# skitzoid/Box2D-MT

Measured on AMD Instinct MI355X. Metric: world steps/sec at 99858 bodies per GPU (BASELINE config 3: Tumbler 100k, CCD off; Step = collide + island solve + broad-phase + state read-back); for N > 1: container-steps/s = world steps/s x N containers in the one sharded world, higher is better.
Workload: dtype f32

## Files before the change

box2d-mt_amd/csrc/b2d_kernels_broadphase.h:

```cpp
#ifndef B2D_KERNELS_BROADPHASE_H
#define B2D_KERNELS_BROADPHASE_H

#include "b2d_kernels_solve_large.h"

#define SYNC_TILE 1024
__global__ __launch_bounds__(256) void k_sync_fixtures(DW W)
{
	b2dPhaseStamp(W);
	DState* S = W.st;
	const int n = W.nProxies;
	const int tid = (int)threadIdx.x;
	__shared__ int s_list[SYNC_TILE];
	__shared__ int s_cnt, s_base;
	const int perLane = n >= 262144 ? SYNC_TILE / 256 : 1, tile = 256 * perLane;
	if (blockIdx.x == 0 && tid == 0) S->c.gridFresh = 0;
	for (int base = blockIdx.x * tile; base < n; base += gridDim.x * tile)
	{
		if (tid == 0) s_cnt = 0;
		__syncthreads();
		for (int j = 0; j < perLane; ++j)
		{
			const int p = base + j * 256 + tid;
			if (p >= n) break;
			const int body = W.p_body[p];
// ... 638 lines not shown
__device__ __forceinline__ bool createBlocked(const DW& W, const DState* S, int smallPath)
{
	if (smallPath && S->c.nPairs > COUNT_RANK_MAX) return true;
	if (!smallPath && (S->c.overflow & 2) != 0) return true;
	return S->c.nContacts + S->c.nNewContacts > W.capContacts;
}

__global__ __launch_bounds__(256) void k_create_contacts(DW W, const uint64_t* keys, const int2* proxies, int smallPath)
{
	b2dPhaseStamp(W);
	DState* S = W.st;
	const int n = S->c.nPairs < W.capPairs ? S->c.nPairs : W.capPairs;
	if (createBlocked(W, S, smallPath)) return;
	const int base = S->c.nContacts;
	const ContactArrays& C = W.ca[S->cur];
	for (int i = blockIdx.x * blockDim.x + threadIdx.x; i < n; i += gridDim.x * blockDim.x)
	{
		if (!W.pairFirst[i]) continue;
		const int dst = base + W.pairRank[i];
		if (dst >= W.capContacts)
		{
			atomicOr(&S->c.overflow, 1);
			continue;
		}
		int2 pr = proxies[i];
		int pA = pr.x, pB = pr.y;
		if (b2dContactSwap(W.shapes[W.p_shape[pA]].type, W.shapes[W.p_shape[pB]].type) == 1)
		{
			int t = pA;
			pA = pB;
// ... 1 lines not shown
		}
		const int bodyA = W.p_body[pA], bodyB = W.p_body[pB];
		const bool sensor = ((W.p_filter1[pA] | W.p_filter1[pB]) & PF_SENSOR) != 0;
		uint32_t flags = CF_ENABLED | (sensor ? CF_SENSOR : 0u);
		if (isToiCandidate(W, pA, pB, bodyA, bodyB))
		{
			flags |= CF_TOI_CANDIDATE;
			const int k = atomicAdd(&S->c.nNewToiCand, 1);
			if (k < TOI_NEW_LIST_MAX) W.toiNewList[k] = dst;
		}
		float2 mA = W.p_mat[pA], mB = W.p_mat[pB];
		float friction = b2dSqrt(mA.x * mB.x);
		float restitution = mA.y > mB.y ? mA.y : mB.y;
		C.ids[dst] = make_int4(pA, pB, bodyA, bodyB);
		C.key[dst] = keys[i];
		C.flags[dst] = flags;
		C.mat[dst] = make_float4(friction, restitution, 0.0f, 1.0f);
		C.man0[dst] = make_float4(0, 0, 0, 0);
		C.man1[dst] = make_float4(0, 0, 0, 0);
		C.imp[dst] = make_float4(0, 0, 0, 0);
		C.man3[dst] = make_int4(0, 0, 0, 0);
		C.color[dst] = -1;
		C.mgr[dst] = -1;
		if (!sensor)
		{
			W.b_wake[bodyA] = 1;
			W.b_wake[bodyB] = 1;
		}
	}
}

__global__ __launch_bounds__(256) void k_create_finish(DW W, int smallPath)
{
	b2dPhaseStamp(W);
	DState* S = W.st;
	if (createBlocked(W, S, smallPath)) return;
	for (int i = blockIdx.x * blockDim.x + threadIdx.x; i < W.nBodies; i += gridDim.x * blockDim.x)
	{
		if (W.b_wake[i])
		{
			W.b_wake[i] = 0;
			const uint32_t f = W.b_flags[i];
			if ((f & BF_AWAKE) != 0 && W.b_pos[i].w == 0.0f) continue;
			W.b_flags[i] = f | BF_AWAKE;
// ... 257 lines not shown
```

box2d-mt_amd/csrc/b2d_kernels_collide.h:

```cpp
#ifndef B2D_KERNELS_COLLIDE_H
#define B2D_KERNELS_COLLIDE_H

#include "b2d_world.h"
#include "b2d_toi.h"

__device__ __forceinline__ Xf loadXf(const float4* b_xf, int body)
{
	float4 t = b_xf[body];
	Xf xf;
	xf.p = v2(t.x, t.y);
	xf.q.s = t.z;
	xf.q.c = t.w;
	return xf;
}

__device__ __forceinline__ AABB loadAabb(const float4* p_fat, int proxy)
{
	float4 t = p_fat[proxy];
	AABB a;
	a.lo = v2(t.x, t.y);
	a.hi = v2(t.z, t.w);
	return a;
}

// ... 690 lines not shown
	for (int i = blockIdx.x * blockDim.x + threadIdx.x; i < n; i += gridDim.x * blockDim.x)
	{
		const int4 ids = C.ids[i];
		const unsigned lo = (unsigned)(ids.z < ids.w ? ids.z : ids.w), hi = (unsigned)(ids.z < ids.w ? ids.w : ids.z);
		const unsigned long long key = ((unsigned long long)lo << 32) | hi;
		int a = 0, b = nPairs;
		while (a < b)
		{
			const int m = (a + b) >> 1;
			if (pairs[m] < key) a = m + 1; else b = m;
		}
		if (a < nPairs && pairs[a] == key) C.flags[i] |= CF_FILTER;
	}
}

__global__ __launch_bounds__(256) void k_compact_contacts(DW W)
{
	b2dPhaseStamp(W);
	DState* S = W.st;
	if (S->c.nDestroy == 0) return;
	const int n = S->c.nContacts;
	const ContactArrays& A = W.ca[S->cur];
	const ContactArrays& B = W.ca[1 - S->cur];
	for (int i = blockIdx.x * blockDim.x + threadIdx.x; i < n; i += gridDim.x * blockDim.x)
	{
		if (W.keepFlag[i])
		{
			int j = W.keepScan[i];
			const uint32_t fl = A.flags[i];
			B.ids[j] = A.ids[i];
			B.key[j] = A.key[i];
			B.flags[j] = fl;
			if ((fl & CF_FOREIGN) == 0)
			{
				B.mat[j] = A.mat[i];
				B.man0[j] = A.man0[i];
				B.man1[j] = A.man1[i];
				B.imp[j] = A.imp[i];
				B.man3[j] = A.man3[i];
			}
			B.color[j] = A.color[i];
			const int m = A.mgr[i];
			B.mgr[j] = m;
			if (m >= 0) W.toiPos2c[m] = j;
		}
	}
	if (b2dLastBlockArrive(W, ARRIVE_COMPACT) && threadIdx.x == 0)
	{
		S->c.nContacts = W.keepScan[n];
		S->cur = 1 - S->cur;
	}
}

__device__ __forceinline__ uint32_t hashKey(uint64_t k)
{
	k ^= k >> 33;
	k *= 0xff51afd7ed558ccdULL;
	k ^= k >> 33;
	k *= 0xc4ceb9fe1a85ec53ULL;
	k ^= k >> 33;
	return (uint32_t)k;
}

__device__ __forceinline__ uint32_t htLiveMask(const DW& W)
{
	const uint32_t want = 4u * (uint32_t)W.st->c.nContacts + 1024u;
	uint32_t m = 0xffffffffu >> __clz((int)(want | 1u));
	return m < W.htMask ? m : W.htMask;
}

__device__ __forceinline__ void htInsert(const DW& W, uint64_t key)
{
	const uint32_t mask = htLiveMask(W);
	uint32_t h = hashKey(key) & mask;
	for (;;)
	{
		unsigned long long old = atomicCAS((unsigned long long*)&W.ht_keys[h], 0ull, (unsigned long long)key);
		if (old == 0ull || old == key) return;
		h = (h + 1) & mask;
	}
}

__device__ __forceinline__ bool htContains(const DW& W, uint64_t key)
{
	const uint32_t mask = htLiveMask(W);
	uint32_t h = hashKey(key) & mask;
	for (;;)
	{
		uint64_t v = W.ht_keys[h];
		if (v == key) return true;
		if (v == 0) return false;
		h = (h + 1) & mask;
	}
}

__global__ __launch_bounds__(256) void k_ht_clear(DW W)
{
	b2dPhaseStamp(W);
	if (W.st->c.nMoves == 0) return;
	for (uint32_t i = blockIdx.x * blockDim.x + threadIdx.x, live = htLiveMask(W); i <= live; i += gridDim.x * blockDim.x)
	{
		W.ht_keys[i] = 0;
	}
}

__global__ __launch_bounds__(256) void k_ht_build(DW W)
{
	b2dPhaseStamp(W);
	DState* S = W.st;
	if (S->c.nMoves == 0) return;
	const int n = S->c.nContacts;
	const ContactArrays& C = W.ca[S->cur];
	for (int i = blockIdx.x * blockDim.x + threadIdx.x; i < n; i += gridDim.x * blockDim.x)
	{
		htInsert(W, C.key[i] + 1ull);
	}
}

#endif
```

box2d-mt_amd/csrc/b2d_kernels_toi.h:

```cpp
#ifndef B2D_KERNELS_TOI_H
#define B2D_KERNELS_TOI_H

#include "b2d_kernels_broadphase.h"
#include "b2d_toi.h"

#define TOI_LANES 512
#define TOI_CAND_MAX 512
#define TOI_MOVES_MAX 128
#define TOI_PAIRS_MAX 512
#define TOI_RECOMP_MAX 512
#define TOI_WOKEN_MAX 256
#define TOI_EVENTS_MAX 100000
#define TOI_NEWPAIR_MAX 256
#define TOI_MOVED_ALL_MAX 32768

__device__ __forceinline__ uint32_t ldFlags(const uint32_t* p)
{
	return __hip_atomic_load(p, __ATOMIC_RELAXED, __HIP_MEMORY_SCOPE_AGENT);
}

__device__ __forceinline__ Sweep loadSweep(const DW& W, int body)
{
	const float4 p0 = W.b_pos0[body], p = W.b_pos[body], m = W.b_mass[body];
	Sweep s;
// ... 1133 lines not shown
		for (int i = tid; i < nPairs; i += LANES)
		{
			if (!s_pairFirst[i] || !s_pairCand[i] || base + s_pairRank[i] >= W.capContacts) continue;
			int before = 0;
			for (int j = 0; j < nPairs; ++j)
			{
				if (s_pairFirst[j] && s_pairCand[j] && s_pairRank[j] < s_pairRank[i]) ++before;
			}
			const int slot = s_toiOrder + before;
			C.mgr[base + s_pairRank[i]] = slot;
			W.toiPos2c[slot] = base + s_pairRank[i];
		}
		__syncthreads();
		if (tid == 0)
		{
			int total = s_nC + s_nNew;
			if (total > W.capContacts) total = W.capContacts;
			s_nC = total;
			s_events += 1;
			int cands = 0;
			for (int j = 0; j < nPairs; ++j) cands += (s_pairFirst[j] && s_pairCand[j] && base + s_pairRank[j] < W.capContacts) ? 1 : 0;
			s_toiOrder += cands;
		}
		__syncthreads();

		}
		const int nB = solid ? s_nBodies : 0;
		TOI_T(7);
		const int nTail = s_nC - nC0;
		for (int bi = 0; bi < nB; ++bi)
// ... 94 lines not shown
```

box2d-mt_amd/csrc/b2d_kernels_toi_chains.h:

```cpp
#ifndef B2D_KERNELS_TOI_CHAINS_H
#define B2D_KERNELS_TOI_CHAINS_H

#include "b2d_kernels_toi.h"

#define CHAIN_LANES 64
#define CHAIN_CAND_MAX 64
#define CHAIN_EVENTS_MAX 4096
#define CHAIN_ADJ_MAX 32
#define TOI_GROUPS_MAX 262144

#define TOI_UNSAFE_PARTNER 1
#define TOI_UNSAFE_WOKE 2
#define TOI_UNSAFE_PAIR 4
#define TOI_UNSAFE_CAPACITY 8
#define TOI_UNSAFE_MOVED 16

__global__ __launch_bounds__(256) void k_toi_groups_begin(DW W)
{
	b2dPhaseStamp(W);
	DState* S = W.st;
	const int n = S->c.nToiList < W.capContacts ? S->c.nToiList : W.capContacts;
	const ContactArrays& C = W.ca[S->cur];
	for (int k = blockIdx.x * blockDim.x + threadIdx.x; k < n; k += gridDim.x * blockDim.x)
	{
// ... 127 lines not shown
			A.mat[i] = B.mat[i];
			A.man0[i] = B.man0[i];
			A.man1[i] = B.man1[i];
			A.imp[i] = B.imp[i];
			A.man3[i] = B.man3[i];
		}
		if (t0 == 0)
		{
			S->c.nToiEvents = 0;
			S->c.nToiMoved = 0;
			S->c.nToiNewPairs = 0;
			S->c.nToiChainCreated = 0;
			S->c.nToiLog = 0;
			S->c.toiIncomplete = 0;
			S->c.spToiStraddle = 0;
			S->c.nContacts = S->c.nContactsSnap;
			S->c.nToiOrder = S->c.nToiOrderSnap;
		}
	}
}

__device__ __forceinline__ void toiChainRun(const DW& W, const StepParams& sp, int haveGrid, int group, int* census)
{
	DState* S = W.st;
	const ContactArrays& C = W.ca[S->cur];
	const int lane = threadIdx.x;
	const int D = W.toiGroups[group];
	const int* adjL = W.toiGroupList + (size_t)group * CHAIN_ADJ_MAX;
	const int nAdj = W.toiGroupCount[group] < CHAIN_ADJ_MAX ? W.toiGroupCount[group] : CHAIN_ADJ_MAX;
	const float4 massD = W.b_mass[D];
// ... 578 lines not shown
				C.color[dst] = -1;
				C.mgr[dst] = -1;
				if (!sensor)
				{
					W.b_pos[bodyA].w = 0.0f;
					W.b_pos[bodyB].w = 0.0f;
					W.b_rowDirty[bodyA] = 1;
					W.b_rowDirty[bodyB] = 1;
				}
			}
			__syncthreads();
			if (threadIdx.x == 0)
			{
				S->c.nContacts = base + s_created;
				S->c.nToiChainCreated = s_created;
			}
		}
	}
}

__global__ __launch_bounds__(CHAIN_LANES) void k_toi_chains(DW W, StepParams sp, int haveGrid)
{
	b2dPhaseStamp(W);
	DState* S = W.st;
	__shared__ int s_chainCensus[2];
	if (threadIdx.x == 0) { s_chainCensus[0] = 0; s_chainCensus[1] = 0; }
	__syncthreads();
	if ((S->c.toiUnsafe & (TOI_UNSAFE_PARTNER | TOI_UNSAFE_CAPACITY)) == 0)
	{
		const int nGroups = S->c.nToiGroups < TOI_GROUPS_MAX ? S->c.nToiGroups : TOI_GROUPS_MAX;
// ... 7 lines not shown
	if (b2dLastBlockArrive(W, ARRIVE_CHAINS, (unsigned)s_chainCensus[0], (unsigned)s_chainCensus[1], &events, &calls))
	{
		if (threadIdx.x == 0)
		{
			if (events) atomicAdd(&S->c.nToiEvents, (int)events);
			if (calls) atomicAdd(&S->c.nToiCalls, (int)calls);
		}
		toiChainsEnd(W);
	}
}

__global__ __launch_bounds__(256) void k_bp_clear(DW W)
{
	b2dPhaseStamp(W);
	DState* S = W.st;
	if (blockIdx.x == 0 && threadIdx.x == 0)
	{
		S->c.nLargeProxies = 0;
		S->c.nLargeMoves = 0;
		S->c.nPairs = 0;
		S->c.nNewContacts = 0;
		S->c.nMovesSeen = S->c.nMoves;
		S->c.gridFresh = S->c.nMoves != 0 ? 1 : 0;
	}
	if (blockIdx.x == 0 && threadIdx.x < 32) S->c.candRounds[threadIdx.x] = 0;
	if (S->c.nMoves == 0) return;
	const uint32_t stride = gridDim.x * blockDim.x, t0 = blockIdx.x * blockDim.x + threadIdx.x;
	{
		const float cap = 4.0f * W.cellSize;
		float ext = 0.0f;
		for (uint32_t p = t0; p < (uint32_t)W.nProxies; p += stride)
		{
// ... 1 lines not shown
			const float4 a = W.p_fat[p];
			const float e = fmaxf(a.z - a.x, a.w - a.y);
			if (e <= cap && e > ext) ext = e;
		}
		blockAtomicMaxIfAbove((int*)&S->c.cellExtBits, ext > 0.0f ? (int)__float_as_uint(ext) : 0);
	}
	{
		const int4 z = make_int4(0, 0, 0, 0);
		int4* gc = (int4*)W.gridCount;
		int4* gu = (int4*)W.gridCursor;
		for (uint32_t i = t0, n4 = (W.gridMask + 1u) >> 2; i < n4; i += stride)
		{
			gc[i] = z;
			gu[i] = z;
		}
		int4* hk = (int4*)W.ht_keys;
		for (uint32_t i = t0, n2 = (htLiveMask(W) + 1u) >> 1; i < n2; i += stride) hk[i] = z;
	}
}

__global__ __launch_bounds__(256) void k_bp_build(DW W)
{
	b2dPhaseStamp(W);
	DState* S = W.st;
	if (S->c.nMoves == 0) return;
	const int stride = gridDim.x * blockDim.x, t0 = blockIdx.x * blockDim.x + threadIdx.x;
	const int nC = S->c.nContacts;
	const ContactArrays& C = W.ca[S->cur];
	for (int i = t0; i < nC; i += stride) if ((C.flags[i] & CF_FOREIGN) == 0) htInsert(W, C.key[i] + 1ull);
	const int n = W.nProxies;
	for (int p = t0; p < n; p += stride)
	{
		if (W.p_body[p] < 0) continue;
		const float4 a = W.p_fat[p];
		if (proxyIsLarge(W, a))
		{
			const int k = atomicAdd(&S->c.nLargeProxies, 1);
			W.largeProxies[k] = p;
		}
		else
		{
			int ix, iy;
			proxyCell(W, a, &ix, &iy);
			atomicAdd(&W.gridCount[cellHash(ix, iy, W.gridMask)], 1);
// ... 6 lines not shown
```

box2d-mt_amd/csrc/b2d_world.h:

```cpp
#ifndef B2D_WORLD_H
#define B2D_WORLD_H

#include "b2d_solver.h"
#include "b2d_joint.h"
#include "b2d_wave.h"

#define BF_TYPE_MASK 0x3u
#define BF_AWAKE 0x4u
#define BF_AUTOSLEEP 0x8u
#define BF_BULLET 0x10u
#define BF_FIXEDROT 0x20u
#define BF_ACTIVE 0x40u
#define BF_ISLAND 0x80u
#define BF_LARGE 0x100u

#define BT_STATIC 0u
#define BT_KINEMATIC 1u
#define BT_DYNAMIC 2u

#define CF_TOUCHING 0x1u
#define CF_ENABLED 0x2u
#define CF_FILTER 0x4u
#define CF_TOI_CANDIDATE 0x8u
#define CF_SENSOR 0x10u
// ... 141 lines not shown
	int collideBlocksDone;
	int chainBlocksDone;
	int edgesBlocksDone;
	int nFreeIslands;
	int nSmallJointed;
	int nStraddle;
	int nStraddleJoints;
	int nResolve;
	int nMigrated;
	int spContacts[SHARD_MAX_RANKS], spJoints[SHARD_MAX_RANKS];
	int spMigBodies[SHARD_MAX_RANKS];
	int spBodies[SHARD_MAX_RANKS], spProxies[SHARD_MAX_RANKS];
	int spToiCreated;
	int spToiStraddle;
	int spOwnRows;
};

struct PreSolveRec
{
	int4 info;
	unsigned long long key;
	unsigned long long pad;
	float4 o0, o1, oimp;
	int4 o3;
	float4 n0, n1, nimp;
	int4 n3;
	float4 mat;
};
struct ToiLogRec
{
// ... 38 lines not shown
struct DW
{
	DState* st;
	uint32_t stampMask;
	int nBodies, nProxies, nJoints, nShapes;
	int capContacts, capPairs, capMoves;
	int serialOrphans;
	int noFreeBodies;
	int testMaxColors, testColorRounds;
	int testSpinMax;
	int restPoll;
	int hubSerial;
	int smallMaxW;
	int bigChunks;
	uint32_t htMask;
	uint32_t gridMask;
	float cellSize, invCellSize;

	float4* b_pos;
	float4* b_pos0;
	float4* b_vel;
	float4* b_xf;
	float4* b_mass;
	float4* b_damp;
	float4* b_force;
	uint32_t* b_flags;
	int* b_wake;
	int* b_order;
	int* orderBody;

// ... 320 lines not shown
```

box2d-mt_amd/csrc/b2hip_api_callbacks.h:

```cpp

int b2hip_set_contact_filter(b2hip_world* w, b2hip_should_collide_fn fn, void* user)
{
	if (int rcu = checkUsable(w, "b2hip_set_contact_filter", true)) return rcu;
	w->filterFn = fn;
	w->filterUser = user;
	w->dw.userFilter = hasFilter(w) ? 1 : 0;
	return B2HIP_OK;
}

int b2hip_set_contact_filter_batch(b2hip_world* w, b2hip_should_collide_batch_fn fn, void* user)
{
	if (int rcu = checkUsable(w, "b2hip_set_contact_filter_batch", true)) return rcu;
	w->filterBatchFn = fn;
	if (fn) w->filterUser = user;
	w->dw.userFilter = hasFilter(w) ? 1 : 0;
	return B2HIP_OK;
}

int b2hip_default_should_collide(b2hip_world* w, int fixture_a, int fixture_b)
{
	if (!w || fixture_a < 0 || fixture_b < 0 || fixture_a >= (int)w->fixtures.size() || fixture_b >= (int)w->fixtures.size())
		return setError(B2HIP_ERR_INVALID, "bad fixture id");
	const HostFixture& a = w->fixtures[fixture_a];
	const HostFixture& b = w->fixtures[fixture_b];
// ... 237 lines not shown
	out->toi_pending_first_pass = w->last.nToiList;
	out->toi_serial_fallbacks = w->toiFallbacks;
	out->blocks = w->last.nBlocks;
	out->cut_constraints = w->last.nCutRows;
	out->block_max_rows = w->last.blkMaxRows;
	out->partitions = w->last.partitions;
	out->block_solver_steps = w->blockSteps;
	out->free_islands = w->last.nFreeIslands;
	out->sweep_solver_steps = w->sweepSteps;
	out->hub_constraints = w->last.nHubRows;
	out->hub_fixpoint_rounds = w->last.hubRounds;
	out->hub_serial_chunks = w->last.hubSerialChunks;
	out->toi_chain_contacts = w->toiChainContacts;
	out->toi_pre_solve_reruns = w->toiPreSolveReruns;
	out->solver_recoveries = w->solverRecoveries + w->colorRecoveries;
	return 0;
}

int b2hip_get_solver_timing(b2hip_world* w, float* ms, double* algorithmic_bytes, int* constraints, int* bodies)
{
	if (!w) return setError(B2HIP_ERR_INVALID, "null world");
	if (ms) *ms = w->solverMs;
	if (algorithmic_bytes) *algorithmic_bytes = w->solverBytes;
	if (constraints) *constraints = w->solverConstraints;
	if (bodies) *bodies = w->solverBodies;
	return 0;
}

int b2hip_set_kernel_timing(b2hip_world* w, int enable)
{
// ... 43 lines not shown
```

box2d-mt_amd/csrc/b2hip_api_snapshot.h:

```cpp

namespace
{
struct SnapHeader
{
	char magic[8];
	uint32_t version, szDState, szHostBody, szHostFixture, szShape, szJoint;
	uint32_t nBodies, nFixtures, nShapes, nJoints, nFree, nContacts, nToiOrder, nMoves;
	uint32_t stateCount, cur;
	int32_t nextNode, leafCount, lastContacts, newFixture;
	float inv_dt0, cellSize;
	int32_t eventsOn, solverHints;
};
const uint32_t kSnapVersion = 5;
const char kSnapMagic[8] = { 'B', '2', 'H', 'I', 'P', 'S', 'N', '1' };

struct SnapWriter
{
	std::vector<char> out;
	void host(const void* p, size_t n) { const char* c = (const char*)p; out.insert(out.end(), c, c + n); }
	int dev(const void* p, size_t n)
	{
		const size_t at = out.size();
		out.resize(at + n);
		if (n == 0) return 0;
// ... 144 lines not shown
	for (size_t k = 0; k < nS; ++k)
	{
		ShapeRec sr;
		memcpy(&sr, shapesAt + k, sizeof(sr));
		if (sr.type < 0 || sr.type > 2 || sr.count < 0 || sr.count > B2D_MAX_POLY_VERTS) return corrupt("shape");
	}
	for (size_t k = 0; k < h.nFree; ++k)
	{
		FreeUnit fu;
		memcpy(&fu, freeAt + k, sizeof(fu));
		if (fu.leaf < -1 || fu.leaf >= h.nextNode) return corrupt("proxy id free list");
	}
	DState ds;
	memcpy(&ds, dsAt, sizeof(ds));
	if (ds.cur != (int)h.cur || ds.c.nContacts != (int)nC || ds.c.nToiOrder != (int)nT || ds.c.nMoves < (int)nM) return corrupt("device state block");

	struct Sec { const void* p; size_t bytes; };
	auto sec = [&](size_t n, size_t elem) { Sec x = { in.take(n * elem), n * elem }; return x; };
	const Sec sPos = sec(nb, 16), sPos0 = sec(nb, 16), sVel = sec(nb, 16), sXf = sec(nb, 16), sMass = sec(nb, 16), sDamp = sec(nb, 16), sForce = sec(nb, 16);
	const Sec sFlags = sec(nb, 4), sWake = sec(nb, 4), sHead = sec(nb, 4), sBlk = sec(nb, 4);
	const Sec sFat = sec(np, 16), sPBody = sec(np, 4), sPShape = sec(np, 4), sPKey = sec(np, 4), sF0 = sec(np, 4), sF1 = sec(np, 4), sPMat = sec(np, 8), sNext = sec(np, 4);
	const Sec cIds = sec(nC, 16), cKey = sec(nC, 8), cFlags = sec(nC, 4), cMat = sec(nC, 16), cMan0 = sec(nC, 16), cMan1 = sec(nC, 16), cImp = sec(nC, 16),
		cMan3 = sec(nC, 16), cColor = sec(nC, 4), cMgr = sec(nC, 4);
	const Sec sToi = sec(nT, 4), sMoves = sec(nM, 4);
	if (!in.ok) return setError(B2HIP_ERR_INVALID, "snapshot truncated");
	auto inRange = [](const Sec& x, long long lo, long long hi)
	{
		const int* v = (const int*)x.p;
		for (size_t i = 0; i < x.bytes / 4; ++i)
		{
// ... 175 lines not shown
```

box2d-mt_amd/csrc/b2hip_api_step.h:

```cpp

int b2hip_step_begin(b2hip_world* w, float dt, int velocity_iterations, int position_iterations)
{
	if (int rc = checkUsable(w, "b2hip_step_begin", false)) return rc;
	if (w->stepActive) return setError(B2HIP_ERR_INVALID, "b2hip_step_begin inside a step (finish it with b2hip_step_end)");
	DEVICE_GUARD(w);
	return stepFailed(w, stepBeginImpl(w, dt, velocity_iterations, position_iterations));
}

static bool keyLess(const std::pair<unsigned long long, int>& a, const std::pair<unsigned long long, int>& b) { return a < b; }

static void toManifold(b2hip_manifold* m, float4 m0, float4 m1, float4 imp, int4 m3)
{
	m->type = m3.z;
	m->point_count = m3.w;
	m->local_normal[0] = m0.x; m->local_normal[1] = m0.y;
	m->local_point[0] = m0.z; m->local_point[1] = m0.w;
	m->point_local[0][0] = m1.x; m->point_local[0][1] = m1.y;
	m->point_local[1][0] = m1.z; m->point_local[1][1] = m1.w;
	m->normal_impulse[0] = imp.x; m->tangent_impulse[0] = imp.y;
	m->normal_impulse[1] = imp.z; m->tangent_impulse[1] = imp.w;
	m->id_key[0] = (uint32_t)m3.x;
	m->id_key[1] = (uint32_t)m3.y;
}

// ... 596 lines not shown
	if (w->debugSync) HIP_TRY(hipStreamSynchronize(w->stream));
	refreshMirror(w);
	const Counters& c = w->h_dstate->c;
	w->lastContacts = c.nContacts;
	w->last.nContacts = c.nContacts;
	w->last.nMoves = c.nMoves;
	if (c.nMovesSeen > 256 && !w->gridForced)
	{
		long long rounds = 0;
		for (int k = 0; k < 32; ++k) rounds += c.candRounds[k];
		const double perProxy = 64.0 * (double)rounds / (double)c.nMovesSeen;
		if (perProxy > 128.0) w->gridHalf = true; else if (perProxy < 48.0) w->gridHalf = false;
		w->dw.gridHalf = w->gridHalf ? 1 : 0;
	}
	w->last.nNewContacts = c.nNewContacts;
	w->last.nPairs = c.nPairs;
	w->last.overflow = c.overflow;
	if (w->colorSmallPending)
	{
		w->colorSmallPending = false;
		w->last.nColors = c.nColors;
		if (c.overflow & 4) return setError(B2HIP_ERR_CAPACITY, "more than 64 constraint colours on one body");
		if (c.nUncolored != 0) return setError(B2HIP_ERR_CAPACITY, "incremental colouring did not converge");
	}
	if ((c.overflow & 0x2040) == 0x2040) return setError(B2HIP_ERR_CAPACITY, "a block of the large-island partition holds more rows or home bodies than its workgroup takes (the census the host partitions by did not see them)");
	if (c.overflow & 64)
	{
		if (w->handoverWhy) handoverPostMortem(w);
		return setError(B2HIP_ERR_HIP, "a wait inside a resident large-island solver timed out (a workgroup was not resident, or a hand-over never came)");
	}
// ... 185 lines not shown
```

box2d-mt_amd/csrc/b2hip_host_phases.h:

```cpp

static int spExchangeState(b2hip_world* w, int mode);
static int spExchangePairs(b2hip_world* w, long long* totalPairs, int* straddling);
static int spResolve(b2hip_world* w, int nVirt = 0);
static int spAfterToi(b2hip_world* w);
static int spBeginStep(b2hip_world* w);

static int radixBits(int maxKey)
{
	int bits = 1;
	while ((1 << bits) <= maxKey && bits < 31) ++bits;
	return bits;
}

static void radixPasses(int first, int bits, std::vector<std::pair<int, int>>& out)
{
	const int passes = (bits + RADIX_BITS - 1) / RADIX_BITS;
	for (int p = 0, at = 0; p < passes; ++p)
	{
		const int width = (bits - at + (passes - p) - 1) / (passes - p);
		out.push_back(std::make_pair(first + at, width));
		at += width;
	}
}

// ... 113 lines not shown

static int findNewContacts(b2hip_world* w, bool sync)
{
	for (int attempt = 0; sync && attempt < 4; ++attempt)
	{
		int rc = findNewContactsOnce(w, true);
		if (rc != 1) return rc;
	}
	if (sync) return setError(B2HIP_ERR_CAPACITY, "pair buffer overflow");
	return findNewContactsOnce(w, false);
}

static int findNewContactsOnce(b2hip_world* w, bool sync)
{
	DW& d = w->dw;
	LAUNCH(w, k_bp_clear, gridFor(std::max(d.htMask, d.gridMask) + 1), 256, d);
	LAUNCH(w, k_bp_build, gridFor(std::max(d.capContacts, d.nProxies)), 256, d);
	deviceExclusiveScan<int>(w->stream, d.gridCount, d.gridStart, d.scanTmp, w->scanCtx, w->consts.p + 1, (int)(d.gridMask + 1));
	LAUNCH(w, k_grid_fill, gridFor(d.nProxies), 256, d, 0);
	if (int rk = ktBracket(w, 4, 7)) return rk;
	if (d.gridHalf) LAUNCH(w, k_find_pairs_window, gridFor((size_t)d.capMoves * 64, 256, 2048), 256, d);
	else LAUNCH(w, k_find_pairs_small, gridFor((size_t)d.capMoves * 64, 256, 2048), 256, d);
	if (int rk = ktBracket(w, 4, 7)) return rk;
	LAUNCH(w, k_find_pairs_large, 1024, 256, d);
	bool large = false;
	if (w->spatial)
	{
		long long total = 0;
		int straddle = 0;
		int rc = spExchangePairs(w, &total, &straddle);
// ... 1253 lines not shown
```

box2d-mt_amd/csrc/b2hip_host_world.h:

```cpp

static thread_local std::string g_lastError;

static int setError(int code, const std::string& msg)
{
	g_lastError = msg;
	return code;
}

#define HIP_TRY(expr)                                                                                   \
	do                                                                                                  \
	{                                                                                                   \
		hipError_t _e = (expr);                                                                         \
		if (_e != hipSuccess)                                                                           \
		{                                                                                               \
			return setError(B2HIP_ERR_HIP, std::string(#expr) + ": " + hipGetErrorString(_e));          \
		}                                                                                               \
	} while (0)

static void (*g_rcclDestroy)(void* comm) = nullptr;

template <typename T>
struct DevArray
{
	T* p = nullptr;
// ... 202 lines not shown
	std::vector<std::pair<int*, size_t> > spTape;
	b2hip_world* spTapeFrom = nullptr;
	size_t spTapeCursor = 0;
	long long spToiRedos = 0;
	size_t spUp = 0;
	DevArray<int> scanFlags;
	ScanFlags scanCtx;
	DevArray<float> stateOut;
	DevArray<int> gridBar;
	int dfEpoch;
	bool noSideStream, profileDetail;
	int collideStage = -1;
	int solidRoundsEnv = 0;
	int collideSplitEnv = -1;
	bool collideUniOff = false;
	int collideSortEnv = -1;
	hipStream_t stream2 = nullptr;
	hipEvent_t evFork = nullptr, evJoin = nullptr;
	DevArray<int> consts;
	DevArray<unsigned long long> filterPairs;
	std::vector<int> nonStatic;
	bool orderDirty = false;
	DevArray<int> b_order, orderBody;
	DevArray<int> bigRoots;
	std::vector<int2> editOps;
	std::vector<int> proxyEdits;
	std::vector<int> fatEdits;
	bool proxyListsStale = false;
	DevArray<int2> d_editOps;
	b2hip_should_collide_fn filterFn = nullptr;
// ... 467 lines not shown
static int envInt(const char* k, int unset) { const char* e = getenv(k); return e ? atoi(e) : unset; }

static void readSwitches(b2hip_world* w)
{
	DW& d = w->dw;
	w->debugSync = envSet("B2HIP_DEBUG");
	w->traceLaunches = envSet("B2HIP_TRACE_LAUNCHES");
	w->debugTrace = envSet("B2HIP_TRACE");
	w->forceLarge = envInt("B2HIP_FORCE_LARGE", 0);
	w->kernelTimingLaunches = envSet("B2HIP_SOLVER_LAUNCHES");
	w->noSideStream = envSet("B2HIP_NO_SIDE_STREAM");
	w->profileDetail = envInt("B2HIP_PROFILE_DETAIL", 1) != 0;
	if (const char* e = getenv("B2HIP_SOLID_ROUNDS")) { const int v = atoi(e); w->solidRoundsEnv = (v == 1 || v == 2 || v == 4 || v == 8) ? v : 0; }
	w->collideSplitEnv = envInt("B2HIP_COLLIDE_SPLIT", -1);
	w->collideUniOff = envInt("B2HIP_COLLIDE_UNI", 1) == 0;
	w->collideSortEnv = envInt("B2HIP_COLLIDE_SORT", -1);
	w->collideStage = envInt("B2HIP_COLLIDE_STAGE", -1);
	w->noSweepBlocks = envSet("B2HIP_NO_SWEEP_BLOCKS");
	w->tracePartition = envSet("B2HIP_TRACE_PARTITION");
	w->traceRecovery = envSet("B2HIP_TRACE_RECOVERY");
	if (const char* e = getenv("B2HIP_GRID_HALF")) { w->gridForced = true; w->gridHalf = atoi(e) != 0; d.gridHalf = w->gridHalf ? 1 : 0; }
	d.noChainCreate = envSet("B2HIP_TOI_NO_CHAIN_CREATE") ? 1 : 0;
	d.noOwnIdBlocks = envSet("B2HIP_NO_OWN_ID_BLOCKS") ? 1 : envSet("B2HIP_OWN_ID_BLOCKS_ALL") ? -1 : 0;
	w->noBlocks = envSet("B2HIP_NO_BLOCKS");
	w->blockLanes = 0;
	if (const char* e = getenv("B2HIP_BLOCK_LANES")) w->blockLanes = atoi(e) == 512 ? 512 : (atoi(e) == 256 ? 256 : (atoi(e) == 1024 ? 1024 : 0));
	w->toiSerialOnly = envSet("B2HIP_TOI_SERIAL");
	w->toiSyncOnly = envSet("B2HIP_TOI_SYNC");
	w->toiDomWideOnly = envSet("B2HIP_TOI_DOM_WIDE");
	w->noToiSpecDomains = envSet("B2HIP_TOI_NO_SPEC_DOMAINS");
// ... 43 lines not shown
	int rc = 0;
#define ENS(arr, n) do { rc = w->arr.ensure((n), s); if (rc) return rc; } while (0)
	ENS(d_state, 1);
	ENS(b_pos, nb); ENS(b_pos0, nb); ENS(b_vel, nb); ENS(b_xf, nb); ENS(b_mass, nb); ENS(b_damp, nb); ENS(b_force, nb);
	ENS(b_flags, nb); ENS(b_wake, nb); ENS(b_rowDirty, nb); ENS(b_order, nb); ENS(orderBody, nb); ENS(bigRoots, SHARD_BIG_MAX);
	ENS(p_fat, np); ENS(p_body, np); ENS(p_shape, np); ENS(p_key, np); ENS(p_filter0, np); ENS(p_filter1, np); ENS(p_mat, np);
	ENS(b_proxyHead, nb); ENS(p_next, np);
	ENS(d_shapes, std::max<size_t>(w->shapes.size(), 1));
	ENS(d_joints, std::max<size_t>(w->joints.size(), 1));
	ENS(d_gears, std::max<size_t>(w->gears.size(), 1));
	ENS(solveSnapJoints, w->recoverOn ? std::max<size_t>(w->joints.size(), 1) : 1); ENS(solveSnapGears, w->recoverOn ? std::max<size_t>(w->gears.size(), 1) : 1);
	ENS(jadjStart, nb + 2); ENS(jadj, 2 * w->joints.size() + 2); ENS(rootJointStart, nb + 2); ENS(rootJointCursor, nb);
	ENS(lj_list, w->joints.size() + 2); ENS(rootJointOkay, nb);
	const size_t capPairs = std::max<size_t>(std::max<size_t>(8 * np + 4096, w->pairKey.cap), w->pairCapHint);
	const size_t capContacts = std::max<size_t>(needContacts + capPairs, 1024);
	for (int k = 0; k < 2; ++k)
	{
		ENS(c_ids[k], capContacts); ENS(c_key[k], capContacts); ENS(c_flags[k], capContacts); ENS(c_mat[k], capContacts);
		ENS(c_man0[k], capContacts); ENS(c_man1[k], capContacts); ENS(c_imp[k], capContacts); ENS(c_man3[k], capContacts);
		ENS(c_color[k], capContacts); ENS(c_mgr[k], capContacts);
	}
	const size_t cc = w->c_ids[0].cap;
	{
		size_t want = (size_t)nextPow2(2 * cc);
		if (w->ht_keys.cap < want)
		{
			rc = w->ht_keys.ensure(want, s, false);
			if (rc) return rc;
		}
	}
	ENS(parent, nb); ENS(rootSeed, nb); ENS(rootBodies, nb); ENS(rootContacts, nb); ENS(rootJoints, nb); ENS(rootIsland, nb);
	ENS(deg, nb + 1); ENS(adjStart, nb + 2); ENS(adjCursor, nb); ENS(adj, 2 * cc); ENS(adjSlot, cc);
	ENS(rootScanIn, nb + 1); ENS(rootScanOut, nb + 2);
	ENS(si_root, nb + 1); ENS(si_bodyStart, nb + 2); ENS(si_contactStart, nb + 2); ENS(si_wStart, nb + 2); ENS(si_maxLevel, nb + 1);
	ENS(si_bodies, nb); ENS(si_contacts, cc); ENS(si_level, cc); ENS(si_stack, nb); ENS(si_lastLevel, nb);
	ENS(b_slot, nb); ENS(b_island, nb); ENS(chunkFirst, (nb + cc) / (TINY_CHUNK_LANES / 2) + 4);
	ENS(li_bodies, nb); ENS(li_contacts, cc); ENS(li_roots, nb); ENS(li_color, cc);
	ENS(colorCount, cc + 2 + COLOR_SLOT_PADDED * COLOR_SLOT_STRIDE); ENS(colorStart, cc + 2); ENS(colorCursor, cc + 2 + COLOR_SLOT_PADDED * COLOR_SLOT_STRIDE); ENS(li_sorted, cc); ENS(li_ref, cc);
	ENS(bodyClaim, nb); ENS(bodyColorMask, nb); ENS(bodyActive, nb); ENS(bodyRest, nb); ENS(b_posv, nb); ENS(evKey, cc); ENS(evInfo, cc); ENS(uncolList, COLOR_SMALL_MAX); ENS(compactList, COLOR_SMALL_MAX); ENS(hubRowOf, cc); ENS(hubList, cc); ENS(hubDelta, cc); ENS(hubMeta, 8); ENS(hubFirst, nb); ENS(solveSnapBody, w->recoverOn ? 6 * nb : 1); ENS(solveSnapImp, w->recoverOn ? cc : 1); ENS(solveSnapCFlags, w->recoverOn ? cc : 1); ENS(rootPen, ROOT_PEN_SLOTS * nb); ENS(rootDone, nb); ENS(rootSleepMin, nb);
	if (w->lc.cap < (size_t)LC_WORDS * cc)
	{
		rc = w->lc.ensure((size_t)LC_WORDS * cc, s, false, false);
		if (rc) return rc;
	}
	if (w->warmDelta.cap < 4 * cc)
// ... 454 lines not shown
```

box2d-mt_amd/python/b2hip.py:

```python
import ctypes as C
import os

import numpy as np

_HERE = os.path.dirname(os.path.abspath(__file__))
LIB_PATH = os.path.join(os.path.dirname(_HERE), "libb2hip.so")

STATIC, KINEMATIC, DYNAMIC = 0, 1, 2
CIRCLE, EDGE, POLYGON = 0, 1, 2
POLYGON_RADIUS = np.float32(2.0) * np.float32(0.005)


class WorldDef(C.Structure):
    _fields_ = [("gravity_x", C.c_float), ("gravity_y", C.c_float), ("allow_sleep", C.c_int),
                ("warm_starting", C.c_int), ("continuous", C.c_int), ("sub_stepping", C.c_int),
                ("auto_clear_forces", C.c_int), ("device", C.c_int)]


class BodyDef(C.Structure):
    _fields_ = [("type", C.c_int), ("px", C.c_float), ("py", C.c_float), ("angle", C.c_float),
                ("vx", C.c_float), ("vy", C.c_float), ("w", C.c_float),
                ("linear_damping", C.c_float), ("angular_damping", C.c_float), ("gravity_scale", C.c_float),
                ("allow_sleep", C.c_int), ("awake", C.c_int), ("fixed_rotation", C.c_int),
                ("bullet", C.c_int), ("active", C.c_int)]
# ... 71 lines not shown
    _fields_ = [("body_a", C.c_int), ("body_b", C.c_int), ("target", C.c_float * 2), ("max_force", C.c_float),
                ("frequency_hz", C.c_float), ("damping_ratio", C.c_float), ("collide_connected", C.c_int)]


class GearJointDef(C.Structure):
    _fields_ = [("joint1", C.c_int), ("joint2", C.c_int), ("ratio", C.c_float), ("collide_connected", C.c_int)]


class Counters(C.Structure):
    _fields_ = [(n, C.c_int32) for n in (
        "bodies", "proxies", "contacts", "touching_contacts", "islands", "small_islands", "large_islands",
        "small_island_bodies", "small_island_contacts", "large_island_bodies", "large_island_contacts",
        "colors", "moved_proxies", "new_contacts", "destroyed_contacts", "solver_chunks",
        "pos_iterations_large", "overflow_flags", "toi_events", "toi_calls", "toi_pending_first_pass", "toi_serial_fallbacks",
        "blocks", "cut_constraints", "block_max_rows", "partitions", "block_solver_steps", "free_islands", "sweep_solver_steps",
        "hub_constraints", "hub_fixpoint_rounds", "hub_serial_chunks", "toi_chain_contacts", "toi_pre_solve_reruns", "solver_recoveries")]


BODY_STATE_DTYPE = np.dtype([("px", "f4"), ("py", "f4"), ("angle", "f4"), ("vx", "f4"), ("vy", "f4"), ("w", "f4"),
                             ("cx", "f4"), ("cy", "f4"), ("flags", "u4"), ("sleep_time", "f4")])

CONTACT_DTYPE = np.dtype([("fixture_a", "i4"), ("fixture_b", "i4"), ("body_a", "i4"), ("body_b", "i4"),
                          ("flags", "u4"), ("manifold_type", "i4"), ("point_count", "i4"),
                          ("local_normal", "f4", 2), ("local_point", "f4", 2), ("point_local", "f4", (2, 2)),
                          ("normal_impulse", "f4", 2), ("tangent_impulse", "f4", 2), ("id_key", "u4", 2),
                          ("friction", "f4"), ("restitution", "f4"), ("tangent_speed", "f4")])

class QueryFilter(C.Structure):
    _fields_ = [("mask", C.c_uint16), ("include_sensors", C.c_int)]


# ... 500 lines not shown
```

include/b2hip.h:

```cpp
#ifndef B2HIP_H
#define B2HIP_H

#include <stddef.h>
#include <stdint.h>

#ifdef __cplusplus
extern "C" {
#endif

typedef struct b2hip_world b2hip_world;

typedef enum b2hip_status
{
	B2HIP_OK = 0,
	B2HIP_ERR_INVALID = -1,
	B2HIP_ERR_HIP = -2,
	B2HIP_ERR_NO_DEVICE = -3,
	B2HIP_ERR_UNSUPPORTED = -4,
	B2HIP_ERR_CAPACITY = -5
} b2hip_status;

enum { B2HIP_STATIC_BODY = 0, B2HIP_KINEMATIC_BODY = 1, B2HIP_DYNAMIC_BODY = 2 };
enum { B2HIP_SHAPE_CIRCLE = 0, B2HIP_SHAPE_EDGE = 1, B2HIP_SHAPE_POLYGON = 2,
       B2HIP_SHAPE_CHAIN = 3 };
// ... 195 lines not shown
	int32_t toi_pending_first_pass;
	int32_t toi_serial_fallbacks;
	int32_t blocks;
	int32_t cut_constraints;
	int32_t block_max_rows;
	int32_t partitions;
	int32_t block_solver_steps;
	int32_t free_islands;
	int32_t sweep_solver_steps;
	int32_t hub_constraints;
	int32_t hub_fixpoint_rounds;
	int32_t hub_serial_chunks;
	int32_t toi_chain_contacts;
	int32_t toi_pre_solve_reruns;
	int32_t solver_recoveries;
} b2hip_counters;

const char* b2hip_last_error(void);
const char* b2hip_version(void);

int b2hip_world_create(const b2hip_world_def* def, b2hip_world** out);
void b2hip_world_destroy(b2hip_world* w);

int b2hip_set_gravity(b2hip_world* w, float gx, float gy);
int b2hip_shift_origin(b2hip_world* w, float x, float y);
int b2hip_set_flags(b2hip_world* w, int allow_sleep, int warm_starting, int continuous, int sub_stepping);

int b2hip_create_body(b2hip_world* w, const b2hip_body_def* def);
int b2hip_create_fixture(b2hip_world* w, int body, const b2hip_fixture_def* def, const b2hip_shape* shape);
int b2hip_create_revolute_joint(b2hip_world* w, const b2hip_revolute_joint_def* def);
// ... 220 lines not shown
```

Before: 349.9.

## Maintain contact-key hash set incrementally instead of rebuilding every step

The contact-key hash table used to be cleared and rebuilt from all contacts on every step with moves. It now persists across steps: new contacts are inserted in k_create_contacts, destroyed contacts become tombstones in k_compact_contacts, and a full rebuild happens only when load, tombstone count or sizing thresholds require it or when TOI/snapshot paths invalidate it. This removes the per-step clear and full insert pass, at the cost of tombstone probe lengths, extra atomics in create, and more complex validity tracking. An optional env-gated checker is added.

```diff
diff --git a/box2d-mt_amd/csrc/b2d_kernels_broadphase.h b/box2d-mt_amd/csrc/b2d_kernels_broadphase.h
--- a/box2d-mt_amd/csrc/b2d_kernels_broadphase.h
+++ b/box2d-mt_amd/csrc/b2d_kernels_broadphase.h
@@ -676,6 +676,19 @@
 	if (createBlocked(W, S, smallPath)) return;
 	const int base = S->c.nContacts;
 	const ContactArrays& C = W.ca[S->cur];
+	__shared__ int s_keyset;
+	if (threadIdx.x == 0)
+	{
+		const Counters& c = S->c;
+		const int64_t used = (int64_t)c.nContacts + (int64_t)c.nNewContacts + (int64_t)c.htTomb - (int64_t)c.htReuse;
+		const bool kept = htKept(W, c);
+		s_keyset = kept && 4 * used <= 3 * ((int64_t)c.htLive + 1) ? 1 : 0;
+		if (kept && !s_keyset) S->c.htValid = 0;
+	}
+	__syncthreads();
+	const bool keyset = s_keyset != 0;
+	const uint32_t mask = S->c.htLive;
+	int reused = 0;
 	for (int i = blockIdx.x * blockDim.x + threadIdx.x; i < n; i += gridDim.x * blockDim.x)
 	{
 		if (!W.pairFirst[i]) continue;
@@ -707,6 +720,7 @@
 		float restitution = mA.y > mB.y ? mA.y : mB.y;
 		C.ids[dst] = make_int4(pA, pB, bodyA, bodyB);
 		C.key[dst] = keys[i];
+		if (keyset && htInsertNew(W, mask, keys[i] + 1ull)) ++reused;
 		C.flags[dst] = flags;
 		C.mat[dst] = make_float4(friction, restitution, 0.0f, 1.0f);
 		C.man0[dst] = make_float4(0, 0, 0, 0);
@@ -721,6 +735,7 @@
 			W.b_wake[bodyB] = 1;
 		}
 	}
+	if (keyset) blockAtomicAddInt2(&S->c.htReuse, reused, &S->c.htReuse, 0);
 }
 
 __global__ __launch_bounds__(256) void k_create_finish(DW W, int smallPath)
diff --git a/box2d-mt_amd/csrc/b2d_kernels_collide.h b/box2d-mt_amd/csrc/b2d_kernels_collide.h
--- a/box2d-mt_amd/csrc/b2d_kernels_collide.h
+++ b/box2d-mt_amd/csrc/b2d_kernels_collide.h
@@ -728,6 +728,137 @@
 	}
 }
 
+#define HT_TOMB 0xffffffffffffffffull
+
+__device__ __forceinline__ uint32_t hashKey(uint64_t k)
+{
+	k ^= k >> 33;
+	k *= 0xff51afd7ed558ccdULL;
+	k ^= k >> 33;
+	k *= 0xc4ceb9fe1a85ec53ULL;
+	k ^= k >> 33;
+	return (uint32_t)k;
+}
+
+__device__ __forceinline__ uint32_t htIdealMask(const DW& W, int n)
+{
+	const uint32_t want = 4u * (uint32_t)n + 1024u;
+	uint32_t m = 0xffffffffu >> __clz((int)(want | 1u));
+	return m < W.htMask ? m : W.htMask;
+}
+
+__device__ __forceinline__ uint32_t htLiveMask(const DW& W) { return W.st->c.htLive; }
+
+__device__ __forceinline__ bool htKept(const DW& W, const Counters& c)
+{
+	return c.htValid != 0 && !W.spatial && !W.userFilter && !W.htAlways;
+}
+
+__device__ __forceinline__ bool htNeedsRebuild(const DW& W, const Counters& c, uint32_t ideal)
+{
+	if (!htKept(W, c)) return true;
+	const uint64_t cur = (uint64_t)c.htLive + 1u;
+	if (ideal > c.htLive) return true;
+	if (cur >= 4u * ((uint64_t)ideal + 1u)) return true;
+	const int64_t used = (int64_t)c.nContacts + (int64_t)c.htTomb - (int64_t)c.htReuse;
+	return 2 * used > (int64_t)cur;
+}
+
+__device__ __forceinline__ void htInsert(const DW& W, uint32_t mask, uint64_t key)
+{
+	uint32_t h = hashKey(key) & mask;
+	for (;;)
+	{
+		unsigned long long old = atomicCAS((unsigned long long*)&W.ht_keys[h], 0ull, (unsigned long long)key);
+		if (old == 0ull || old == key) return;
+		h = (h + 1) & mask;
+	}
+}
+
+__device__ __forceinline__ bool htInsertNew(const DW& W, uint32_t mask, uint64_t key)
+{
+	uint32_t h = hashKey(key) & mask;
+	for (;;)
+	{
+		unsigned long long v = W.ht_keys[h];
+		while (v == 0ull || v == HT_TOMB)
+		{
+			const unsigned long long old = atomicCAS((unsigned long long*)&W.ht_keys[h], v, (unsigned long long)key);
+			if (old == v) return v == HT_TOMB;
+			v = old;
+		}
+		h = (h + 1) & mask;
+	}
+}
+
+__device__ __forceinline__ bool htErase(const DW& W, uint32_t mask, uint64_t key)
+{
+	uint32_t h = hashKey(key) & mask;
+	for (;;)
+	{
+		const uint64_t v = W.ht_keys[h];
+		if (v == key)
+		{
+			W.ht_keys[h] = HT_TOMB;
+			return true;
+		}
+		if (v == 0) return false;
+		h = (h + 1) & mask;
+	}
+}
+
+__device__ __forceinline__ bool htContains(const DW& W, uint64_t key)
+{
+	const uint32_t mask = htLiveMask(W);
+	uint32_t h = hashKey(key) & mask;
+	for (;;)
+	{
+		uint64_t v = W.ht_keys[h];
+		if (v == key) return true;
+		if (v == 0) return false;
+		h = (h + 1) & mask;
+	}
+}
+
+__global__ __launch_bounds__(256) void k_ht_check_count(DW W)
+{
+	b2dPhaseStamp(W);
+	DState* S = W.st;
+	if (!htKept(W, S->c)) return;
+	const uint32_t mask = S->c.htLive;
+	const int n = S->c.nContacts;
+	const ContactArrays& C = W.ca[S->cur];
+	int missing = 0, own = 0, slots = 0, tombs = 0;
+	for (int i = blockIdx.x * blockDim.x + threadIdx.x; i < n; i += gridDim.x * blockDim.x)
+	{
+		if ((C.flags[i] & CF_FOREIGN) != 0) continue;
+		++own;
+		if (!htContains(W, C.key[i] + 1ull)) ++missing;
+	}
+	for (uint32_t i = blockIdx.x * blockDim.x + threadIdx.x; i <= mask; i += gridDim.x * blockDim.x)
+	{
+		const uint64_t v = W.ht_keys[i];
+		if (v == HT_TOMB) ++tombs;
+		else if (v != 0) ++slots;
+	}
+	blockAtomicAddInt2(&S->c.htMismatch, missing, &S->c.htChkSlots, slots);
+	blockAtomicAddInt2(&S->c.htChkTomb, tombs, &S->c.htChkOwn, own);
+}
+
+__global__ void k_ht_check_total(DW W)
+{
+	b2dPhaseStamp(W);
+	Counters& c = W.st->c;
+	if (htKept(W, c))
+	{
+		if (c.htChkSlots != c.htChkOwn) c.htMismatch += 1;
+		if (c.htChkTomb != c.htTomb - c.htReuse) c.htMismatch += 1;
+	}
+	c.htChkSlots = 0;
+	c.htChkTomb = 0;
+	c.htChkOwn = 0;
+}
+
 __global__ __launch_bounds__(256) void k_compact_contacts(DW W)
 {
 	b2dPhaseStamp(W);
@@ -736,9 +867,16 @@
 	const int n = S->c.nContacts;
 	const ContactArrays& A = W.ca[S->cur];
 	const ContactArrays& B = W.ca[1 - S->cur];
+	const bool keyset = htKept(W, S->c);
+	const uint32_t mask = S->c.htLive;
+	int tombs = 0;
 	for (int i = blockIdx.x * blockDim.x + threadIdx.x; i < n; i += gridDim.x * blockDim.x)
 	{
-		if (W.keepFlag[i])
+		if (!W.keepFlag[i])
+		{
+			if (keyset && (A.flags[i] & CF_FOREIGN) == 0 && htErase(W, mask, A.key[i] + 1ull)) ++tombs;
+		}
+		else
 		{
 			int j = W.keepScan[i];
 			const uint32_t fl = A.flags[i];
@@ -759,6 +897,7 @@
 			if (m >= 0) W.toiPos2c[m] = j;
 		}
 	}
+	if (keyset) blockAtomicAddInt2(&S->c.htTomb, tombs, &S->c.htTomb, 0);
 	if (b2dLastBlockArrive(W, ARRIVE_COMPACT) && threadIdx.x == 0)
 	{
 		S->c.nContacts = W.keepScan[n];
@@ -766,69 +905,4 @@
 	}
 }
 
-__device__ __forceinline__ uint32_t hashKey(uint64_t k)
-{
-	k ^= k >> 33;
-	k *= 0xff51afd7ed558ccdULL;
-	k ^= k >> 33;
-	k *= 0xc4ceb9fe1a85ec53ULL;
-	k ^= k >> 33;
-	return (uint32_t)k;
-}
-
-__device__ __forceinline__ uint32_t htLiveMask(const DW& W)
-{
-	const uint32_t want = 4u * (uint32_t)W.st->c.nContacts + 1024u;
-	uint32_t m = 0xffffffffu >> __clz((int)(want | 1u));
-	return m < W.htMask ? m : W.htMask;
-}
-
-__device__ __forceinline__ void htInsert(const DW& W, uint64_t key)
-{
-	const uint32_t mask = htLiveMask(W);
-	uint32_t h = hashKey(key) & mask;
-	for (;;)
-	{
-		unsigned long long old = atomicCAS((unsigned long long*)&W.ht_keys[h], 0ull, (unsigned long long)key);
-		if (old == 0ull || old == key) return;
-		h = (h + 1) & mask;
-	}
-}
-
-__device__ __forceinline__ bool htContains(const DW& W, uint64_t key)
-{
-	const uint32_t mask = htLiveMask(W);
-	uint32_t h = hashKey(key) & mask;
-	for (;;)
-	{
-		uint64_t v = W.ht_keys[h];
-		if (v == key) return true;
-		if (v == 0) return false;
-		h = (h + 1) & mask;
-	}
-}
-
-__global__ __launch_bounds__(256) void k_ht_clear(DW W)
-{
-	b2dPhaseStamp(W);
-	if (W.st->c.nMoves == 0) return;
-	for (uint32_t i = blockIdx.x * blockDim.x + threadIdx.x, live = htLiveMask(W); i <= live; i += gridDim.x * blockDim.x)
-	{
-		W.ht_keys[i] = 0;
-	}
-}
-
-__global__ __launch_bounds__(256) void k_ht_build(DW W)
-{
-	b2dPhaseStamp(W);
-	DState* S = W.st;
-	if (S->c.nMoves == 0) return;
-	const int n = S->c.nContacts;
-	const ContactArrays& C = W.ca[S->cur];
-	for (int i = blockIdx.x * blockDim.x + threadIdx.x; i < n; i += gridDim.x * blockDim.x)
-	{
-		htInsert(W, C.key[i] + 1ull);
-	}
-}
-
 #endif
diff --git a/box2d-mt_amd/csrc/b2d_kernels_toi.h b/box2d-mt_amd/csrc/b2d_kernels_toi.h
--- a/box2d-mt_amd/csrc/b2d_kernels_toi.h
+++ b/box2d-mt_amd/csrc/b2d_kernels_toi.h
@@ -1171,6 +1171,7 @@
 		__syncthreads();
 		if (tid == 0)
 		{
+			if (s_nNew) S->c.htValid = 0;
 			int total = s_nC + s_nNew;
 			if (total > W.capContacts) total = W.capContacts;
 			s_nC = total;
diff --git a/box2d-mt_amd/csrc/b2d_kernels_toi_chains.h b/box2d-mt_amd/csrc/b2d_kernels_toi_chains.h
--- a/box2d-mt_amd/csrc/b2d_kernels_toi_chains.h
+++ b/box2d-mt_amd/csrc/b2d_kernels_toi_chains.h
@@ -165,6 +165,7 @@
 			S->c.nToiLog = 0;
 			S->c.toiIncomplete = 0;
 			S->c.spToiStraddle = 0;
+			if (S->c.nContacts != S->c.nContactsSnap) S->c.htValid = 0;
 			S->c.nContacts = S->c.nContactsSnap;
 			S->c.nToiOrder = S->c.nToiOrderSnap;
 		}
@@ -773,6 +774,7 @@
 			{
 				S->c.nContacts = base + s_created;
 				S->c.nToiChainCreated = s_created;
+				if (s_created) S->c.htValid = 0;
 			}
 		}
 	}
@@ -810,8 +812,12 @@
 {
 	b2dPhaseStamp(W);
 	DState* S = W.st;
+	const uint32_t htIdeal = htIdealMask(W, S->c.nContacts);
+	const bool htRebuild = htNeedsRebuild(W, S->c, htIdeal);
 	if (blockIdx.x == 0 && threadIdx.x == 0)
 	{
+		S->c.htBuild = htRebuild && S->c.nMoves != 0 ? 1 : 0;
+		S->c.htNext = htIdeal;
 		S->c.nLargeProxies = 0;
 		S->c.nLargeMoves = 0;
 		S->c.nPairs = 0;
@@ -843,8 +849,11 @@
 			gc[i] = z;
 			gu[i] = z;
 		}
-		int4* hk = (int4*)W.ht_keys;
-		for (uint32_t i = t0, n2 = (htLiveMask(W) + 1u) >> 1; i < n2; i += stride) hk[i] = z;
+		if (htRebuild)
+		{
+			int4* hk = (int4*)W.ht_keys;
+			for (uint32_t i = t0, n2 = (htIdeal + 1u) >> 1; i < n2; i += stride) hk[i] = z;
+		}
 	}
 }
 
@@ -856,7 +865,19 @@
 	const int stride = gridDim.x * blockDim.x, t0 = blockIdx.x * blockDim.x + threadIdx.x;
 	const int nC = S->c.nContacts;
 	const ContactArrays& C = W.ca[S->cur];
-	for (int i = t0; i < nC; i += stride) if ((C.flags[i] & CF_FOREIGN) == 0) htInsert(W, C.key[i] + 1ull);
+	if (S->c.htBuild)
+	{
+		const uint32_t mask = S->c.htNext;
+		for (int i = t0; i < nC; i += stride) if ((C.flags[i] & CF_FOREIGN) == 0) htInsert(W, mask, C.key[i] + 1ull);
+		if (t0 == 0)
+		{
+			S->c.htLive = mask;
+			S->c.htValid = W.spatial || W.userFilter || W.htAlways ? 0 : 1;
+			S->c.htTomb = 0;
+			S->c.htReuse = 0;
+			S->c.htRebuilds += 1;
+		}
+	}
 	const int n = W.nProxies;
 	for (int p = t0; p < n; p += stride)
 	{
diff --git a/box2d-mt_amd/csrc/b2d_world.h b/box2d-mt_amd/csrc/b2d_world.h
--- a/box2d-mt_amd/csrc/b2d_world.h
+++ b/box2d-mt_amd/csrc/b2d_world.h
@@ -179,6 +179,15 @@
 	int spToiCreated;
 	int spToiStraddle;
 	int spOwnRows;
+	uint32_t htLive;
+	int htValid;
+	int htTomb;
+	int htReuse;
+	int htBuild;
+	uint32_t htNext;
+	int htRebuilds;
+	int htMismatch;
+	int htChkSlots, htChkTomb, htChkOwn;
 };
 
 struct PreSolveRec
@@ -247,6 +256,7 @@
 	int smallMaxW;
 	int bigChunks;
 	uint32_t htMask;
+	int htAlways;
 	uint32_t gridMask;
 	float cellSize, invCellSize;
 
diff --git a/box2d-mt_amd/csrc/b2hip_api_callbacks.h b/box2d-mt_amd/csrc/b2hip_api_callbacks.h
--- a/box2d-mt_amd/csrc/b2hip_api_callbacks.h
+++ b/box2d-mt_amd/csrc/b2hip_api_callbacks.h
@@ -275,6 +275,8 @@
 	out->toi_chain_contacts = w->toiChainContacts;
 	out->toi_pre_solve_reruns = w->toiPreSolveReruns;
 	out->solver_recoveries = w->solverRecoveries + w->colorRecoveries;
+	out->keyset_rebuilds = w->last.htRebuilds;
+	out->keyset_mismatches = w->last.htMismatch;
 	return 0;
 }
 
diff --git a/box2d-mt_amd/csrc/b2hip_api_snapshot.h b/box2d-mt_amd/csrc/b2hip_api_snapshot.h
--- a/box2d-mt_amd/csrc/b2hip_api_snapshot.h
+++ b/box2d-mt_amd/csrc/b2hip_api_snapshot.h
@@ -182,6 +182,7 @@
 	DState ds;
 	memcpy(&ds, dsAt, sizeof(ds));
 	if (ds.cur != (int)h.cur || ds.c.nContacts != (int)nC || ds.c.nToiOrder != (int)nT || ds.c.nMoves < (int)nM) return corrupt("device state block");
+	ds.c.htValid = 0;
 
 	struct Sec { const void* p; size_t bytes; };
 	auto sec = [&](size_t n, size_t elem) { Sec x = { in.take(n * elem), n * elem }; return x; };
diff --git a/box2d-mt_amd/csrc/b2hip_api_step.h b/box2d-mt_amd/csrc/b2hip_api_step.h
--- a/box2d-mt_amd/csrc/b2hip_api_step.h
+++ b/box2d-mt_amd/csrc/b2hip_api_step.h
@@ -634,6 +634,8 @@
 		w->dw.gridHalf = w->gridHalf ? 1 : 0;
 	}
 	w->last.nNewContacts = c.nNewContacts;
+	w->last.htRebuilds = c.htRebuilds;
+	w->last.htMismatch = c.htMismatch;
 	w->last.nPairs = c.nPairs;
 	w->last.overflow = c.overflow;
 	if (w->colorSmallPending)
diff --git a/box2d-mt_amd/csrc/b2hip_host_phases.h b/box2d-mt_amd/csrc/b2hip_host_phases.h
--- a/box2d-mt_amd/csrc/b2hip_host_phases.h
+++ b/box2d-mt_amd/csrc/b2hip_host_phases.h
@@ -151,6 +151,11 @@
 static int findNewContactsOnce(b2hip_world* w, bool sync)
 {
 	DW& d = w->dw;
+	if (w->keysetCheck)
+	{
+		LAUNCH(w, k_ht_check_count, gridFor(std::max(d.htMask, (uint32_t)d.capContacts) + 1), 256, d);
+		LAUNCH(w, k_ht_check_total, 1, 1, d);
+	}
 	LAUNCH(w, k_bp_clear, gridFor(std::max(d.htMask, d.gridMask) + 1), 256, d);
 	LAUNCH(w, k_bp_build, gridFor(std::max(d.capContacts, d.nProxies)), 256, d);
 	deviceExclusiveScan<int>(w->stream, d.gridCount, d.gridStart, d.scanTmp, w->scanCtx, w->consts.p + 1, (int)(d.gridMask + 1));
diff --git a/box2d-mt_amd/csrc/b2hip_host_world.h b/box2d-mt_amd/csrc/b2hip_host_world.h
--- a/box2d-mt_amd/csrc/b2hip_host_world.h
+++ b/box2d-mt_amd/csrc/b2hip_host_world.h
@@ -240,6 +240,7 @@
 	int solidRoundsEnv = 0;
 	int collideSplitEnv = -1;
 	bool collideUniOff = false;
+	bool keysetCheck = false;
 	int collideSortEnv = -1;
 	hipStream_t stream2 = nullptr;
 	hipEvent_t evFork = nullptr, evJoin = nullptr;
@@ -737,6 +738,8 @@
 	if (const char* e = getenv("B2HIP_SOLID_ROUNDS")) { const int v = atoi(e); w->solidRoundsEnv = (v == 1 || v == 2 || v == 4 || v == 8) ? v : 0; }
 	w->collideSplitEnv = envInt("B2HIP_COLLIDE_SPLIT", -1);
 	w->collideUniOff = envInt("B2HIP_COLLIDE_UNI", 1) == 0;
+	d.htAlways = envOn("B2HIP_KEYSET_REBUILD") ? 1 : 0;
+	w->keysetCheck = envOn("B2HIP_KEYSET_CHECK");
 	w->collideSortEnv = envInt("B2HIP_COLLIDE_SORT", -1);
 	w->collideStage = envInt("B2HIP_COLLIDE_STAGE", -1);
 	w->noSweepBlocks = envSet("B2HIP_NO_SWEEP_BLOCKS");
@@ -810,6 +813,7 @@
 	ENS(lj_list, w->joints.size() + 2); ENS(rootJointOkay, nb);
 	const size_t capPairs = std::max<size_t>(std::max<size_t>(8 * np + 4096, w->pairKey.cap), w->pairCapHint);
 	const size_t capContacts = std::max<size_t>(needContacts + capPairs, 1024);
+	const void* const keyArrays[3] = {w->ht_keys.p, w->c_key[0].p, w->c_key[1].p};
 	for (int k = 0; k < 2; ++k)
 	{
 		ENS(c_ids[k], capContacts); ENS(c_key[k], capContacts); ENS(c_flags[k], capContacts); ENS(c_mat[k], capContacts);
@@ -825,6 +829,8 @@
 			if (rc) return rc;
 		}
 	}
+	if (keyArrays[0] != w->ht_keys.p || keyArrays[1] != w->c_key[0].p || keyArrays[2] != w->c_key[1].p)
+		HIP_TRY(hipMemsetAsync(&w->d_state.p->c.htValid, 0, sizeof(int), s));
 	ENS(parent, nb); ENS(rootSeed, nb); ENS(rootBodies, nb); ENS(rootContacts, nb); ENS(rootJoints, nb); ENS(rootIsland, nb);
 	ENS(deg, nb + 1); ENS(adjStart, nb + 2); ENS(adjCursor, nb); ENS(adj, 2 * cc); ENS(adjSlot, cc);
 	ENS(rootScanIn, nb + 1); ENS(rootScanOut, nb + 2);
diff --git a/box2d-mt_amd/python/b2hip.py b/box2d-mt_amd/python/b2hip.py
--- a/box2d-mt_amd/python/b2hip.py
+++ b/box2d-mt_amd/python/b2hip.py
@@ -109,7 +109,8 @@
         "colors", "moved_proxies", "new_contacts", "destroyed_contacts", "solver_chunks",
         "pos_iterations_large", "overflow_flags", "toi_events", "toi_calls", "toi_pending_first_pass", "toi_serial_fallbacks",
         "blocks", "cut_constraints", "block_max_rows", "partitions", "block_solver_steps", "free_islands", "sweep_solver_steps",
-        "hub_constraints", "hub_fixpoint_rounds", "hub_serial_chunks", "toi_chain_contacts", "toi_pre_solve_reruns", "solver_recoveries")]
+        "hub_constraints", "hub_fixpoint_rounds", "hub_serial_chunks", "toi_chain_contacts", "toi_pre_solve_reruns", "solver_recoveries",
+        "keyset_rebuilds", "keyset_mismatches")]
 
 
 BODY_STATE_DTYPE = np.dtype([("px", "f4"), ("py", "f4"), ("angle", "f4"), ("vx", "f4"), ("vy", "f4"), ("w", "f4"),
diff --git a/include/b2hip.h b/include/b2hip.h
--- a/include/b2hip.h
+++ b/include/b2hip.h
@@ -233,6 +233,8 @@
 	int32_t toi_chain_contacts;
 	int32_t toi_pre_solve_reruns;
 	int32_t solver_recoveries;
+	int32_t keyset_rebuilds;
+	int32_t keyset_mismatches;
 } b2hip_counters;
 
 const char* b2hip_last_error(void);
```

Result: no change. 357.1, median of 6 (+2.0%).
